# Fireflies-17/Speech-Inpainting

Hardware: AMD Instinct MI355X
Metric: real-time factor (audio-sec/wall-sec) per GPU, 4 s clips @16 kHz, 200 ms mask (higher is better)
Workload: dtype encoder GEMMs and attention products: bf16 MFMA, fp32 accumulate (softmax, LayerNorm, head, arg-max in fp32); vocoder: fp16 MFMA (operands rounded to fp16, saturating), fp32 accumulate, activations stored as fp16; 1 GPU; BASELINE configs[1]: batch=32 x 4 s clips per GPU, 200 ms mask, HuBERT-base + HiFi-GAN V1; step = masked log-mel front-end -> encoder -> arg-max/splice -> vocoder on resident raw clips; global_batch=32, clip_samples=64000, mask_frames=10, parallelism=utterance-sharded x1

## Files before the change

speech_inpainting_amd/csrc/reschain.hip:

```cpp
#include <algorithm>
#include <cstdio>
#include <cstdlib>
#include <type_traits>

#include "common.h"

typedef float f32x4 __attribute__((ext_vector_type(4)));
typedef unsigned int u32x4 __attribute__((ext_vector_type(4)));
typedef unsigned int u32x2 __attribute__((ext_vector_type(2)));
typedef _Float16 f16x8 __attribute__((ext_vector_type(8)));
typedef _Float16 f16x4 __attribute__((ext_vector_type(4)));

#ifdef RPW_TIMELINE
__device__ unsigned long long rc_tl[10];
#define RC_TL_DECL unsigned long long tl_t = wall_clock64(); unsigned long long tl_acc[8] = {0, 0, 0, 0, 0, 0, 0, 0}; unsigned long long tl_tiles = 0; unsigned long long tl_w = 0;
#define RC_TL_W0 tl_w = wall_clock64();
#define RC_TL_W1(ph) tl_acc[ph] += wall_clock64() - tl_w;
#define RC_TL(ph) { const unsigned long long n_ = wall_clock64(); tl_acc[ph] += n_ - tl_t; tl_t = n_; }
#define RC_TL_TILE ++tl_tiles;
#define RC_TL_FLUSH if (threadIdx.x == 0) { for (int q_ = 0; q_ < 8; ++q_) atomicAdd(&rc_tl[q_], tl_acc[q_]); atomicAdd(&rc_tl[8], tl_tiles); atomicAdd(&rc_tl[9], 1ull); }
extern "C" int si_debug_rc_timeline(unsigned long long* out, int reset) {
    if (hipMemcpyFromSymbol(out, HIP_SYMBOL(rc_tl), sizeof(rc_tl)) != hipSuccess) return -1;
    if (reset) { unsigned long long z[10] = {}; if (hipMemcpyToSymbol(HIP_SYMBOL(rc_tl), z, sizeof(z)) != hipSuccess) return -1; }
    return 0;
}
#else
#define RC_TL_DECL
#define RC_TL_W0
#define RC_TL_W1(ph)
#define RC_TL(ph)
#define RC_TL_TILE
#define RC_TL_FLUSH
#endif

namespace {

constexpr int RC_C = 32, RC_ROWB = 64, RC_NW = 8, RC_NT = 64 * RC_NW;
constexpr int RC_RT = 6;
constexpr int RC_R = RC_NW * RC_RT * 16;
constexpr int RC_MARG = 32;
constexpr int RC_KMAX = 11;
constexpr int RC_XBYTES = RC_R * RC_ROWB;
constexpr int RC_ABYTES = (RC_R + 2 * RC_MARG) * RC_ROWB;
constexpr int RC_WBYTES = RC_KMAX * RC_C * RC_ROWB;
constexpr int RC_LDS = RC_XBYTES + RC_ABYTES + 2 * RC_WBYTES + 6 * RC_C * 4;
constexpr int RC_WSLOTS = (RC_WBYTES / 16 + RC_NT - 1) / RC_NT;
constexpr int RC_YSLOTS = RC_R * 4 / RC_NT;
static_assert(RC_R * 4 % RC_NT == 0, "tile staging map");

__device__ __forceinline__ int rc_swz(int row) { return ((row >> 1) & 3) << 4; }

}

template <bool ACC, bool VL>
__global__ __launch_bounds__(RC_NT, 1) void reschain_kernel(const ResChainParams p) {
    extern __shared__ __attribute__((aligned(16))) char smem[];
    char* const Xs = smem;
    char* const As = smem + RC_XBYTES;
    char* const W1s = As + RC_ABYTES;
    char* const W2s = W1s + RC_WBYTES;
    float* const Bs = reinterpret_cast<float*>(W2s + RC_WBYTES);

    __builtin_amdgcn_s_setreg((0 << 11) | (23 << 6) | 1, 1);
    const int tid = threadIdx.x, lane = tid & 63, wave = tid >> 6;
    const int r16 = lane & 15, kg = lane >> 4;
    const int wm0 = wave * (RC_RT * 16);
    const int k = p.k, c = (k - 1) / 2;
    const int H = c * (p.dil[0] + p.dil[1] + p.dil[2] + 3);
    const int Rout = RC_R - 2 * H;
    const int tiles_x = (p.L + Rout - 1) / Rout;
    const int total = VL ? p.total_tiles : tiles_x * p.B;
    auto tile_of = [&](int t, int& tb, int& tm0, int& tL) {
        if constexpr (VL) { const SiVlTile v = si_vl_tile(p.lens, p.B, Rout, t); tb = v.b; tm0 = v.row0; tL = v.L; }
        else { tb = t / tiles_x; tm0 = (t - tb * tiles_x) * Rout; tL = p.L; }
    };
    const int wbytes = k * RC_C * RC_ROWB;

    u32x4 rw[RC_WSLOTS];
    auto issueW = [&](const unsigned short* w) {
        const __amdgpu_buffer_rsrc_t rs = __builtin_amdgcn_make_buffer_rsrc(const_cast<unsigned short*>(w), 0, wbytes, 0x00020000);
// ... 61 lines not shown
            const int lin = lin0 + (tap - c) * dd * RC_ROWB;
            const char* ap = As + (lin ^ ((lin >> 3) & 0x30));
#pragma unroll
            for (int i = 0; i < RC_RT; ++i) y[i] = *reinterpret_cast<const f16x8*>(ap + i * (16 * RC_ROWB));
            const char* wp = Wc + tap * (RC_C * RC_ROWB) + preW;
#pragma unroll
            for (int j = 0; j < 2; ++j) w[j] = *reinterpret_cast<const f16x8*>(wp + j * (16 * RC_ROWB));
        };
        auto mma = [&](const f16x8 (&y)[RC_RT], const f16x8 (&w)[2]) {
#ifdef RC_ABLATE_HALF
            if (wave >= 4) return;
#endif
#ifdef RC_ABLATE_MFMA
#pragma unroll
            for (int i = 0; i < RC_RT; ++i) acc[i][0] += __builtin_bit_cast(f32x4, y[i]);
            acc[0][1] += __builtin_bit_cast(f32x4, w[0]) + __builtin_bit_cast(f32x4, w[1]);
            return;
#endif
#pragma unroll
            for (int i = 0; i < RC_RT; ++i)
#pragma unroll
                for (int j = 0; j < 2; ++j) acc[i][j] = __builtin_amdgcn_mfma_f32_16x16x32_f16(w[j], y[i], acc[i][j], 0, 0, 0);
        };
        f16x8 ya[RC_RT], wa[2], yb[RC_RT], wb[2];
        load(ya, wa, 0);
        for (int tap = 0; tap < k; tap += 2) {
            load(yb, wb, tap + 1 < k ? tap + 1 : k - 1);
            __builtin_amdgcn_sched_barrier(0);
            __builtin_amdgcn_s_setprio(1);
            mma(ya, wa);
            __builtin_amdgcn_s_setprio(0);
            __builtin_amdgcn_sched_barrier(0);
            load(ya, wa, tap + 2 < k ? tap + 2 : k - 1);
            __builtin_amdgcn_sched_barrier(0);
            if (tap + 1 < k) {
                __builtin_amdgcn_s_setprio(1);
                mma(yb, wb);
                __builtin_amdgcn_s_setprio(0);
            }
            __builtin_amdgcn_sched_barrier(0);
        }
    };

    RC_TL_DECL
    for (int tile = blockIdx.x; tile < total; tile += gridDim.x) {
        const int nxt = tile + (int)gridDim.x < total ? tile + (int)gridDim.x : tile;
        int b, tm0, Lb;
        tile_of(tile, b, tm0, Lb);
        const int g0 = tm0 - H;
        const long seg = (long)b * p.L * RC_C;
        const __amdgpu_buffer_rsrc_t orsrc = __builtin_amdgcn_make_buffer_rsrc(p.out16 + seg, 0, Lb * RC_C * 2, 0x00020000);
        const bool edge = g0 < 0 || g0 + RC_R > Lb;

#pragma unroll
        for (int i = 0; i < RC_YSLOTS; ++i) {
            const int q = tid + i * RC_NT;
            const int r = q >> 2, ch = q & 3;
            f16x8 h = __builtin_bit_cast(f16x8, ry[i]);
            *reinterpret_cast<f16x8*>(Xs + r * RC_ROWB + ((ch << 4) ^ rc_swz(r))) = h;
            h = __builtin_elementwise_max(h, h * (_Float16)0.1f);
            const int ra = r + RC_MARG;
            *reinterpret_cast<f16x8*>(As + ra * RC_ROWB + ((ch << 4) ^ rc_swz(ra))) = h;
        }
        __syncthreads();
        RC_TL(0)

        u32x2 prev[ACC ? RC_RT : 1][2];
        auto swap_halves = [&](u32x2& p0, u32x2& p1) {
#pragma unroll
            for (int q = 0; q < 2; ++q) {
                const auto r = __builtin_amdgcn_permlane16_swap(p0[q], p1[q], false, false);
                p0[q] = r[0]; p1[q] = r[1];
            }
        };
        auto chunk_off = [&](int ip, int j, int shift) {
            const int r = wm0 + 16 * (2 * ip + (kg & 1)) + r16 + shift;
            return r * RC_ROWB + ((((2 * j + (kg >> 1)) << 4)) ^ rc_swz(r));
        };
        auto epi1 = [&](auto maskc) {
            constexpr bool MASK = decltype(maskc)::value;
#pragma unroll
            for (int ip = 0; ip < RC_RT / 2; ++ip) {
                float inside[2] = {1.f, 1.f};
                if constexpr (MASK) {
#pragma unroll
                    for (int u = 0; u < 2; ++u) { const int g = g0 + wm0 + 16 * (2 * ip + u) + r16; inside[u] = (g >= 0 && g < Lb) ? 1.f : 0.f; }
                }
#pragma unroll
                for (int j = 0; j < 2; ++j) {
                    u32x2 pk[2];
#pragma unroll
                    for (int u = 0; u < 2; ++u) {
                        f16x4 hv;
#pragma unroll
                        for (int e = 0; e < 4; ++e) {
                            float v = si_lrelu01(acc[2 * ip + u][j][e]);
                            if constexpr (MASK) v *= inside[u];
                            hv[e] = (_Float16)v;
                        }
                        pk[u] = __builtin_bit_cast(u32x2, hv);
                    }
                    swap_halves(pk[0], pk[1]);
                    *reinterpret_cast<u32x4*>(As + chunk_off(ip, j, RC_MARG)) = u32x4{pk[0][0], pk[0][1], pk[1][0], pk[1][1]};
                }
            }
        };
        auto epi2 = [&](auto maskc, auto lastc) {
            constexpr bool MASK = decltype(maskc)::value, LAST = decltype(lastc)::value;
            constexpr int HP = (RC_RT / 2 + 1) / 2;
#pragma unroll
            for (int h = 0; h < 2; ++h) {
                const int ip0 = h * HP, ip1 = h == 0 ? HP : RC_RT / 2;
                f16x4 xr[HP][2][2];
#pragma unroll
                for (int ip = ip0; ip < ip1; ++ip)
#pragma unroll
                    for (int u = 0; u < 2; ++u)
// ... 124 lines not shown
```

speech_inpainting_amd/csrc/respair.hip:

```cpp
#include <algorithm>
#include <cstdio>
#include <cstdlib>
#include <type_traits>

#include "common.h"

typedef float f32x4 __attribute__((ext_vector_type(4)));
typedef unsigned int u32x4 __attribute__((ext_vector_type(4)));
typedef unsigned int u32x2 __attribute__((ext_vector_type(2)));
typedef _Float16 f16x8 __attribute__((ext_vector_type(8)));
typedef _Float16 f16x4 __attribute__((ext_vector_type(4)));

constexpr int RPN_HALO = 50;

template <int ROWB>
__device__ __forceinline__ int rpn_swz(int row) {
    if constexpr (ROWB == 128) return (row & 7) << 4;
    else return ((row >> 1) & 3) << 4;
}

template <int C, int R1, int WARPS_M, int TPS, bool ACC, bool VL>
__global__ __launch_bounds__(64 * WARPS_M, 2) void respair_kernel(const ResPairParams p) {
    static_assert(R1 == WARPS_M * 64 && (C == 32 || C == 64), "64-row wave tiles over all C channels");
    constexpr int NT = 64 * WARPS_M;
    constexpr int ROWB = C * 2;
    constexpr int ROWBO = C * 4;
    constexpr int CPR = C / 8;
    constexpr int KS = C / 32;
    constexpr int TN = C / 16;
    constexpr int YPAD = C == 64 ? 32 : 0;
    constexpr int YS = ROWB + YPAD;
    constexpr int YBYTES = (R1 + RPN_HALO) * YS;
    constexpr int WBYTES = TPS * C * ROWB;
    constexpr int WSLOTS = (WBYTES / 16 + NT - 1) / NT;
    constexpr int YRPP = NT / CPR;
    constexpr int YSLOTS = (R1 + RPN_HALO + YRPP - 1) / YRPP;
    constexpr int OXM = (C / 4 - 1) < 15 ? (C / 4 - 1) : 15;
    static_assert(R1 * ROWBO <= YBYTES + 2 * WBYTES, "the output image reuses the operand region (not the biases behind it)");

    __builtin_amdgcn_s_setreg((0 << 11) | (23 << 6) | 1, 1);
    extern __shared__ __attribute__((aligned(16))) char smem[];
    char* const Ys = smem;
    char* const Ws = smem + YBYTES;
    float* const Bs = reinterpret_cast<float*>(smem + YBYTES + 2 * WBYTES);

    const int tid = threadIdx.x, lane = tid & 63, wave = tid >> 6;
    const int r16 = lane & 15, kg = lane >> 4;
    const int wm0 = wave * 64;
    const int k = p.k, d = p.dil;
    const int p1 = d * (k - 1) / 2, p2 = (k - 1) / 2;
    const int BMo = R1 - (k - 1);
    const int R0 = R1 + (k - 1) * d;
    const int tiles_x = (p.L + BMo - 1) / BMo;
    const int total = VL ? p.total_tiles : tiles_x * p.B;
    auto tile_of = [&](int t, int& tb, int& tm0, int& tL) {
        if constexpr (VL) { const SiVlTile v = si_vl_tile(p.lens, p.B, BMo, t); tb = v.b; tm0 = v.row0; tL = v.L; }
        else { tb = t / tiles_x; tm0 = (t - tb * tiles_x) * BMo; tL = p.L; }
    };
    const __amdgpu_buffer_rsrc_t w1rsrc = __builtin_amdgcn_make_buffer_rsrc(const_cast<unsigned short*>(p.w1), 0, k * C * C * 2, 0x00020000);
    const __amdgpu_buffer_rsrc_t w2rsrc = __builtin_amdgcn_make_buffer_rsrc(const_cast<unsigned short*>(p.w2), 0, k * C * C * 2, 0x00020000);

    const int NS1 = (k + TPS - 1) / TPS, NS = 2 * NS1;
    u32x4 rw[WSLOTS];
    auto issueW = [&](int s) {
        const bool second = s >= NS1;
        const int soff = __builtin_amdgcn_readfirstlane((second ? s - NS1 : s) * WBYTES);
#pragma unroll
        for (int i = 0; i < WSLOTS; ++i)
            rw[i] = __builtin_amdgcn_raw_buffer_load_b128(second ? w2rsrc : w1rsrc, (tid + i * NT) * 16, soff, 0);
    };
    auto storeW = [&](char* dst) {
#pragma unroll
        for (int i = 0; i < WSLOTS; ++i) {
            const int q = tid + i * NT;
            if (WBYTES / 16 % NT == 0 || q < WBYTES / 16) {
                const int r = q / CPR, c = q - r * CPR;
                *reinterpret_cast<u32x4*>(dst + r * ROWB + ((c << 4) ^ rpn_swz<ROWB>(r))) = rw[i];
            }
        }
    };

    const int yc = tid % CPR, yr0 = tid / CPR;
    u32x4 ry[YSLOTS];
    auto issueY = [&](int t) {
        int tb, tm0, tL;
        tile_of(t, tb, tm0, tL);
        const int trow0 = tm0 - p2 - p1;
        const __amdgpu_buffer_rsrc_t rs = __builtin_amdgcn_make_buffer_rsrc(const_cast<unsigned short*>(p.y16 + (long)tb * p.L * C), 0, tL * C * 2, 0x00020000);
#pragma unroll
        for (int i = 0; i < YSLOTS; ++i)
            ry[i] = __builtin_amdgcn_raw_buffer_load_b128(rs, ((trow0 + yr0 + i * YRPP) * C + 8 * yc) * 2, 0, 0);
    };

    issueW(0);
    issueY(blockIdx.x);
    if (tid < C / 2) {
        const int which = tid / (C / 4), c4 = (tid % (C / 4)) * 4;
        *reinterpret_cast<f32x4*>(Bs + which * C + c4) = *reinterpret_cast<const f32x4*>((which ? p.b2 : p.b1) + c4);
    }

  for (int tile = blockIdx.x; tile < total; tile += gridDim.x) {
    const int nxt = tile + (int)gridDim.x < total ? tile + (int)gridDim.x : tile;
    int b, m0, Lb;
    tile_of(tile, b, m0, Lb);
    const int t_row0 = m0 - p2;
    const long seg = (long)b * p.L * C;
    const __amdgpu_buffer_rsrc_t yrsrc = __builtin_amdgcn_make_buffer_rsrc(const_cast<unsigned short*>(p.y16 + seg), 0, Lb * C * 2, 0x00020000);
    const __amdgpu_buffer_rsrc_t orsrc = __builtin_amdgcn_make_buffer_rsrc(p.out16 + seg, 0, Lb * C * 2, 0x00020000);

    storeW(Ws);
    issueW(1);
#pragma unroll
    for (int i = 0; i < YSLOTS; ++i) {
        const int r = yr0 + i * YRPP;
        if ((i + 1) * YRPP <= R1 || r < R0) {
            f16x8 h = __builtin_bit_cast(f16x8, ry[i]);
            h = __builtin_elementwise_max(h, h * (_Float16)0.1f);
            *reinterpret_cast<f16x8*>(Ys + r * YS + (YPAD ? yc << 4 : (yc << 4) ^ rpn_swz<ROWB>(r))) = h;
        }
    }
    __syncthreads();

    f32x4 acc[4][TN];
    auto init_acc = [&](const float* bias) {
#pragma unroll
        for (int j = 0; j < TN; ++j) {
            const f32x4 bv = *reinterpret_cast<const f32x4*>(bias + 16 * j + 4 * kg);
#pragma unroll
            for (int i = 0; i < 4; ++i) acc[i][j] = bv;
        }
    };
    init_acc(Bs);
    const int lin0 = (wm0 + r16) * YS + (kg << 4);
    int preW[KS];
#pragma unroll
    for (int ks = 0; ks < KS; ++ks) preW[ks] = r16 * ROWB + (rpn_swz<ROWB>(r16) ^ (kg << 4) ^ (ks * 64));
    auto compute = [&](int tap0, bool second, int ntap, const char* Wc) {
        const int nsteps = ntap * KS;
        auto load = [&](f16x8 (&y)[4], f16x8 (&w)[TN], int q, const int ks) {
            const int tl = KS == 1 ? q : q >> 1;
            const int soff = (second ? tap0 + tl : (tap0 + tl) * d) * YS + ks * 64;
            const int lin = lin0 + soff;
            const char* yp = Ys + (YPAD ? lin : lin ^ ((lin >> 3) & 0x30));
#pragma unroll
            for (int i = 0; i < 4; ++i) y[i] = *reinterpret_cast<const f16x8*>(yp + i * (16 * YS));
            const char* wp = Wc + tl * (C * ROWB) + preW[ks];
#pragma unroll
            for (int j = 0; j < TN; ++j) w[j] = *reinterpret_cast<const f16x8*>(wp + j * (16 * ROWB));
        };
        auto mma = [&](const f16x8 (&y)[4], const f16x8 (&w)[TN]) {
#pragma unroll
            for (int i = 0; i < 4; ++i)
#pragma unroll
                for (int j = 0; j < TN; ++j) acc[i][j] = __builtin_amdgcn_mfma_f32_16x16x32_f16(w[j], y[i], acc[i][j], 0, 0, 0);
        };
        f16x8 ya[4], wa[TN], yb[4], wb[TN];
        load(ya, wa, 0, 0);
        for (int q = 0; q < nsteps; q += 2) {
            load(yb, wb, q + 1 < nsteps ? q + 1 : nsteps - 1, KS - 1);
            __builtin_amdgcn_sched_barrier(0);
            __builtin_amdgcn_s_setprio(1);
            mma(ya, wa);
            __builtin_amdgcn_s_setprio(0);
            __builtin_amdgcn_sched_barrier(0);
            load(ya, wa, q + 2 < nsteps ? q + 2 : nsteps - KS, 0);
            __builtin_amdgcn_sched_barrier(0);
            if (q + 1 < nsteps) {
                __builtin_amdgcn_s_setprio(1);
                mma(yb, wb);
                __builtin_amdgcn_s_setprio(0);
            }
            __builtin_amdgcn_sched_barrier(0);
        }
    };

    for (int s = 0; s < NS; ++s) {
        const bool second = s >= NS1;
        const int q = second ? s - NS1 : s;
        const int tap0 = q * TPS;
        if (s == NS - 1) {
            issueW(0);
            if constexpr (!ACC) issueY(nxt);
        }
        compute(tap0, second, min(TPS, k - tap0), Ws + (s & 1) * WBYTES);
        if (s == NS1 - 1) {
            __syncthreads();
            auto epi1 = [&](auto edge_tag) {
                constexpr bool EDGE = decltype(edge_tag)::value;
#pragma unroll
            for (int ip = 0; ip < 2; ++ip) {
                float inside[2];
#pragma unroll
                for (int u = 0; u < 2; ++u) {
                    const int grow = t_row0 + wm0 + 16 * (2 * ip + u) + r16;
                    inside[u] = (!EDGE || (grow >= 0 && grow < Lb)) ? 1.f : 0.f;
                }
                const int ms = wm0 + 16 * (2 * ip + (kg & 1)) + r16;
#pragma unroll
                for (int j = 0; j < TN; ++j) {
                    u32x2 pk[2];
#pragma unroll
                    for (int u = 0; u < 2; ++u) {
                        f16x4 hv;
#pragma unroll
                        for (int e = 0; e < 4; ++e) hv[e] = (_Float16)(EDGE ? si_lrelu01(acc[2 * ip + u][j][e]) * inside[u] : si_lrelu01(acc[2 * ip + u][j][e]));
                        pk[u] = __builtin_bit_cast(u32x2, hv);
                    }
#pragma unroll
                    for (int q = 0; q < 2; ++q) {
                        const auto r = __builtin_amdgcn_permlane16_swap(pk[0][q], pk[1][q], false, false);
                        pk[0][q] = r[0]; pk[1][q] = r[1];
                    }
                    const int ch = 2 * j + (kg >> 1);
                    *reinterpret_cast<u32x4*>(Ys + ms * YS + (YPAD ? ch << 4 : (ch << 4) ^ rpn_swz<ROWB>(ms))) = u32x4{pk[0][0], pk[0][1], pk[1][0], pk[1][1]};
                }
            }
            };
            if (t_row0 >= 0 && t_row0 + R1 <= Lb) epi1(std::false_type{});
            else epi1(std::true_type{});
            init_acc(Bs + C);
        }
        if (s + 1 < NS) {
            storeW(Ws + ((s + 1) & 1) * WBYTES);
            if (s + 2 < NS) issueW(s + 2);
        }
        __syncthreads();
    }

    constexpr int ORPP = NT / CPR;
    constexpr int OPASS = R1 / ORPP;
    const int c8 = tid % CPR, or0 = tid / CPR;
    u32x4 res[OPASS], prev[ACC ? OPASS : 1];
    int goff[OPASS];
#pragma unroll
    for (int it = 0; it < OPASS; ++it) {
        const int o = or0 + it * ORPP;
        const int grow = m0 + o;
        goff[it] = (o < BMo && grow < Lb) ? (grow * C + 8 * c8) * 2 : (int)0x80000000;
        res[it] = __builtin_amdgcn_raw_buffer_load_b128(yrsrc, goff[it], 0, 0);
        if constexpr (ACC) prev[it] = __builtin_amdgcn_raw_buffer_load_b128(orsrc, goff[it], 0, 0);
    }
#pragma unroll
    for (int i = 0; i < 4; ++i) {
        const int m = wm0 + 16 * i + r16;
#pragma unroll
        for (int j = 0; j < TN; ++j) {
            const int co = 4 * j + kg;
            *reinterpret_cast<f32x4*>(smem + m * ROWBO + ((co ^ (m & OXM)) << 4)) = acc[i][j];
        }
    }
    __syncthreads();
    {
#pragma unroll
        for (int it = 0; it < OPASS; ++it) {
            const int o = or0 + it * ORPP;
            const f32x4 a0 = *reinterpret_cast<const f32x4*>(smem + o * ROWBO + (((2 * c8) ^ (o & OXM)) << 4));
            const f32x4 a1 = *reinterpret_cast<const f32x4*>(smem + o * ROWBO + (((2 * c8 + 1) ^ (o & OXM)) << 4));
            const f16x8 rh = __builtin_bit_cast(f16x8, res[it]);
            f16x8 ph = {};
            if constexpr (ACC) ph = __builtin_bit_cast(f16x8, prev[it]);
            f16x8 out;
#pragma unroll
            for (int e = 0; e < 8; ++e) {
                const float a = e < 4 ? a0[e] : a1[e - 4];
                float v = (a + (float)rh[e]) * p.alpha;
                if constexpr (ACC) v += (float)ph[e];
                out[e] = (_Float16)v;
            }
            __builtin_amdgcn_raw_buffer_store_b128(__builtin_bit_cast(u32x4, out), orsrc, goff[it], 0, 0);
        }
    }
    if constexpr (ACC) issueY(nxt);
    __syncthreads();
  }
}

template <int C, int R1, int WARPS_M, int TPS>
static int respair_launch(si_ctx* ctx, const ResPairParams& p, hipStream_t st) {
    const int BMo = R1 - (p.k - 1);
    const size_t lds = (size_t)(R1 + RPN_HALO) * (C * 2 + (C == 64 ? 32 : 0)) + 2 * (size_t)TPS * C * C * 2 + 2 * (size_t)C * 4;
    const bool vl = p.lens != nullptr;
    auto kern = vl ? (p.accumulate ? respair_kernel<C, R1, WARPS_M, TPS, true, true> : respair_kernel<C, R1, WARPS_M, TPS, false, true>)
                   : (p.accumulate ? respair_kernel<C, R1, WARPS_M, TPS, true, false> : respair_kernel<C, R1, WARPS_M, TPS, false, false>);
    if (int rc = si_ensure_dyn_lds(ctx, reinterpret_cast<const void*>(kern), lds)) return rc;
    const int total = vl ? (int)si_vl_tiles(p.lens_host, p.B, BMo) : ((p.L + BMo - 1) / BMo) * p.B;
    if (total <= 0) return SI_OK;
    ResPairParams pk = p;
    pk.total_tiles = total;
    const int grid = std::min(total, si_num_cus(ctx) * (WARPS_M == 4 ? 2 : 1));
    char name[48];
    snprintf(name, sizeof(name), p.accumulate ? "respair_f16_c%d_acc" : "respair_f16_c%d", C);
    double rows = (double)p.B * p.L;
    if (vl) { rows = 0; for (int b = 0; b < p.B; ++b) rows += p.lens_host[b]; }
    const double elems = rows * C;
    si_prof_begin(ctx, name, 2.0 * 2.0 * elems * C * p.k, elems * (2.0 + 2.0 + (p.accumulate ? 2.0 : 0.0)) + 2.0 * 2.0 * p.k * C * C, st);
    hipLaunchKernelGGL(kern, dim3(grid), dim3(64 * WARPS_M), lds, st, pk);
    si_prof_end(ctx, st);
    SI_HIP_CHECK(hipGetLastError());
    return SI_OK;
}

int si_launch_respair(si_ctx* ctx, int C, const unsigned short* y16, unsigned short* out16, const void* w1, const void* w2,
                      const float* b1, const float* b2, int B, int L, int k, int dil, float alpha, int accumulate, hipStream_t st,
                      const int32_t* lens, const int32_t* lens_host, float out_slope) {
    if ((C != 32 && C != 64 && C != 128 && C != 256) || k < 3 || k > 11 || (k & 1) == 0 || (k - 1) * dil > 50 ||
        ((long)L + 1024) * C * 2 >= (1L << 31)) return 1;
    if (!b1 || !b2) return 1;
    if ((lens == nullptr) != (lens_host == nullptr)) return si_fail(ctx, SI_EINVAL, "respair: ragged batches need the lengths on the device and on the host");
    ResPairParams p{y16, out16, static_cast<const unsigned short*>(w1), static_cast<const unsigned short*>(w2), b1, b2, B, L, k, dil, alpha, accumulate, lens, lens_host, 0, out_slope};
    if (out_slope != 1.f && C < 128) return 1;
    if (C >= 128) return si_launch_respair_wide(ctx, C, p, st);
    return C == 32 ? respair_launch<32, 256, 4, 11>(ctx, p, st) : respair_launch<64, 512, 8, 4>(ctx, p, st);
}
```

speech_inpainting_amd/csrc/respair_wide.hip:

```cpp
#include <algorithm>
#include <cstdio>
#include <cstdlib>

#include "common.h"

typedef float f32x4 __attribute__((ext_vector_type(4)));
typedef unsigned int u32x4 __attribute__((ext_vector_type(4)));
typedef unsigned int u32x2 __attribute__((ext_vector_type(2)));
typedef _Float16 f16x8 __attribute__((ext_vector_type(8)));
typedef _Float16 f16x4 __attribute__((ext_vector_type(4)));

template <int ROWB>
__device__ __forceinline__ int swz16(int row) {
    if constexpr (ROWB >= 256) return (row & 7) << 5;
    else return ((row >> 1) & 3) << 5;
}

#ifdef RPW_TIMELINE
__device__ unsigned long long rpw_tl[2][10];
#define RPW_TL_DECL unsigned long long tl_t = wall_clock64(); unsigned long long tl_acc[6] = {0, 0, 0, 0, 0, 0}; unsigned long long tl_tiles = 0; unsigned long long tl_w = 0, tl_sub[2] = {0, 0};
#define RPW_TL_W0 tl_w = wall_clock64();
#define RPW_TL_W1(q) tl_sub[q] += wall_clock64() - tl_w;
#define RPW_TL(ph) { const unsigned long long n_ = wall_clock64(); tl_acc[ph] += n_ - tl_t; tl_t = n_; }
#define RPW_TL_TILE ++tl_tiles;
#define RPW_TL_FLUSH if (threadIdx.x == 0) { for (int q_ = 0; q_ < 6; ++q_) atomicAdd(&rpw_tl[C == 256][q_], tl_acc[q_]); atomicAdd(&rpw_tl[C == 256][6], tl_tiles); atomicAdd(&rpw_tl[C == 256][7], 1ull); atomicAdd(&rpw_tl[C == 256][8], tl_sub[0]); atomicAdd(&rpw_tl[C == 256][9], tl_sub[1]); }
extern "C" int si_debug_rpw_timeline(unsigned long long* out, int reset) {
    if (hipMemcpyFromSymbol(out, HIP_SYMBOL(rpw_tl), sizeof(rpw_tl)) != hipSuccess) return -1;
    if (reset) { unsigned long long z[2][10] = {}; if (hipMemcpyToSymbol(HIP_SYMBOL(rpw_tl), z, sizeof(z)) != hipSuccess) return -1; }
    return 0;
}
#else
#define RPW_TL_DECL
#define RPW_TL_W0
#define RPW_TL_W1(q)
#define RPW_TL(ph)
#define RPW_TL_TILE
#define RPW_TL_FLUSH
#endif

constexpr int RPW_HALO = 50;

template <int C, int R1, int WARPS_M, int WARPS_N, int BKW, bool ACC, bool VL>
__global__ __launch_bounds__(64 * WARPS_M * WARPS_N, 2) void respair_wide_kernel(const ResPairParams p) {
    static_assert((WARPS_M * WARPS_N == 8 || WARPS_M * WARPS_N == 4) && R1 == WARPS_M * 64 && C == WARPS_N * 64, "64 x 64 wave tiles");
    static_assert(BKW == 128 || BKW == 64, "weight-slab depth");
    constexpr int NT = 64 * WARPS_M * WARPS_N;
    constexpr int ROWBY = C * 2;
    constexpr int ROWBW = BKW * 2;
    constexpr int ROWBO = C * 4;
    constexpr int CPRY = C / 8, CPRW = BKW / 8;
    constexpr int NCH = C / BKW;
    constexpr int KS = BKW / 32;
    constexpr int YBYTES = (R1 + RPW_HALO) * ROWBY;
    constexpr int WBYTES = C * ROWBW;
    constexpr int WSLOTS = C * CPRW / NT;
    constexpr int YSLOTS = ((R1 + RPW_HALO) * CPRY + NT - 1) / NT;
    constexpr int YRPP = NT / CPRY, WRPP = NT / CPRW;
    static_assert(C * CPRW % NT == 0 && NT % CPRY == 0 && NT % CPRW == 0, "staging maps");
    static_assert(R1 * ROWBO <= YBYTES + 2 * WBYTES, "the output image reuses the operand region (not the biases behind it)");

    __builtin_amdgcn_s_setreg((0 << 11) | (23 << 6) | 1, 1);
    extern __shared__ __attribute__((aligned(16))) char smem[];
    char* const Ys = smem;
    char* const Ws = smem + YBYTES;
    float* const Bs = reinterpret_cast<float*>(smem + YBYTES + 2 * WBYTES);

    const int tid = threadIdx.x, lane = tid & 63, wave = tid >> 6;
    const int r16 = lane & 15, kg = lane >> 4;
    const int wm0 = (wave / WARPS_N) * 64, wn0 = (wave % WARPS_N) * 64;
    const int k = p.k, d = p.dil;
    const int p1 = d * (k - 1) / 2, p2 = (k - 1) / 2;
    const int BMo = R1 - (k - 1);
    const int R0 = R1 + (k - 1) * d;
    const int tiles_x = (p.L + BMo - 1) / BMo;
    const int total = VL ? p.total_tiles : tiles_x * p.B;
    auto tile_of = [&](int t, int& tb, int& tm0, int& tL) {
        if constexpr (VL) { const SiVlTile v = si_vl_tile(p.lens, p.B, BMo, t); tb = v.b; tm0 = v.row0; tL = v.L; }
        else { tb = t / tiles_x; tm0 = (t - tb * tiles_x) * BMo; tL = p.L; }
    };
    const __amdgpu_buffer_rsrc_t w1rsrc = __builtin_amdgcn_make_buffer_rsrc(const_cast<unsigned short*>(p.w1), 0, k * C * C * 2, 0x00020000);
    const __amdgpu_buffer_rsrc_t w2rsrc = __builtin_amdgcn_make_buffer_rsrc(const_cast<unsigned short*>(p.w2), 0, k * C * C * 2, 0x00020000);

    const int NS1 = k * NCH, NS = 2 * NS1;
    const int wc = tid % CPRW, wr0 = tid / CPRW;
    u32x4 rw[WSLOTS];
    auto issueW1 = [&](int s, int i) {
        const bool second = s >= NS1;
        const int q = second ? s - NS1 : s;
        const int tap = q / NCH, ch = q - tap * NCH;
        const int soff = __builtin_amdgcn_readfirstlane((tap * C * C + ch * BKW) * 2);
        const int n = wr0 + i * WRPP;
        rw[i] = __builtin_amdgcn_raw_buffer_load_b128(second ? w2rsrc : w1rsrc, (n * C + 8 * wc) * 2, soff, 0);
    };
    auto issueW = [&](int s) {
#pragma unroll
        for (int i = 0; i < WSLOTS; ++i) issueW1(s, i);
    };
    auto storeW1 = [&](char* dst, int i) {
        const int n = wr0 + i * WRPP;
        *reinterpret_cast<u32x4*>(dst + n * ROWBW + ((wc << 4) ^ swz16<ROWBW>(n))) = rw[i];
    };
    auto storeW = [&](char* dst) {
#pragma unroll
        for (int i = 0; i < WSLOTS; ++i) storeW1(dst, i);
    };
    const int yc = tid % CPRY, yr0 = tid / CPRY;
    u32x4 ry[YSLOTS];
    auto issueY = [&](int t) {
        int tb, tm0, tL;
        tile_of(t, tb, tm0, tL);
        const int trow0 = tm0 - p2 - p1;
        const __amdgpu_buffer_rsrc_t rs = __builtin_amdgcn_make_buffer_rsrc(const_cast<unsigned short*>(p.y16 + (long)tb * p.L * C), 0, tL * C * 2, 0x00020000);
#pragma unroll
        for (int i = 0; i < YSLOTS; ++i)
            ry[i] = __builtin_amdgcn_raw_buffer_load_b128(rs, ((trow0 + yr0 + i * YRPP) * C + 8 * yc) * 2, 0, 0);
    };

    if (tid < C / 2) {
        const int which = tid / (C / 4), c4 = (tid % (C / 4)) * 4;
        *reinterpret_cast<f32x4*>(Bs + which * C + c4) = *reinterpret_cast<const f32x4*>((which ? p.b2 : p.b1) + c4);
    }
    const int preW = (wn0 + r16) * ROWBW + (swz16<ROWBW>(wn0 + r16) ^ (kg << 4));
    issueW(0);
    issueY(blockIdx.x);
    RPW_TL_DECL

  for (int tile = blockIdx.x; tile < total; tile += gridDim.x) {
    const int nxt = tile + (int)gridDim.x < total ? tile + (int)gridDim.x : tile;
    int b, m0, Lb;
    tile_of(tile, b, m0, Lb);
    const int t_row0 = m0 - p2;
    const long seg = (long)b * p.L * C;
    const __amdgpu_buffer_rsrc_t yrsrc = __builtin_amdgcn_make_buffer_rsrc(const_cast<unsigned short*>(p.y16 + seg), 0, Lb * C * 2, 0x00020000);
    const __amdgpu_buffer_rsrc_t orsrc = __builtin_amdgcn_make_buffer_rsrc(p.out16 + seg, 0, Lb * C * 2, 0x00020000);

    storeW(Ws);
    issueW(1);
#pragma unroll
    for (int i = 0; i < YSLOTS; ++i) {
        const int r = yr0 + i * YRPP;
        if ((i + 1) * YRPP <= R1 || r < R0) {
            f16x8 h = __builtin_bit_cast(f16x8, ry[i]);
            h = __builtin_elementwise_max(h, h * (_Float16)0.1f);
            *reinterpret_cast<f16x8*>(Ys + r * ROWBY + ((yc << 4) ^ swz16<ROWBY>(r))) = h;
        }
    }
    __syncthreads();
    RPW_TL(0)

    f32x4 acc[4][4];
    auto init_acc = [&](const float* bias) {
#pragma unroll
        for (int j = 0; j < 4; ++j) {
            const f32x4 bv = *reinterpret_cast<const f32x4*>(bias + wn0 + 16 * j + 4 * kg);
#pragma unroll
            for (int i = 0; i < 4; ++i) acc[i][j] = bv;
        }
    };
    init_acc(Bs);
    auto compute = [&](int roff, int cb16, const char* Wc, auto&& hook) {
        const int r0 = wm0 + r16 + roff;
        const int preY = r0 * ROWBY + (swz16<ROWBY>(r0) ^ (kg << 4));
        auto load = [&](f16x8 (&y)[4], f16x8 (&w)[4], int ks) {
            const char* yp = Ys + (preY ^ (cb16 + ks * 64));
            const char* wp = Wc + (preW ^ (ks * 64));
#pragma unroll
            for (int i = 0; i < 4; ++i) y[i] = *reinterpret_cast<const f16x8*>(yp + i * (16 * ROWBY));
#pragma unroll
            for (int j = 0; j < 4; ++j) w[j] = *reinterpret_cast<const f16x8*>(wp + j * (16 * ROWBW));
        };
        auto mma = [&](const f16x8 (&y)[4], const f16x8 (&w)[4]) {
#pragma unroll
            for (int i = 0; i < 4; ++i)
#pragma unroll
                for (int j = 0; j < 4; ++j) acc[i][j] = __builtin_amdgcn_mfma_f32_16x16x32_f16(w[j], y[i], acc[i][j], 0, 0, 0);
        };
        f16x8 ya[4], wa[4], yb[4], wb[4];
        load(ya, wa, 0);
#pragma unroll
        for (int ks = 0; ks < KS; ks += 2) {
            load(yb, wb, ks + 1);
            __builtin_amdgcn_sched_barrier(0);
            __builtin_amdgcn_s_setprio(1);
            mma(ya, wa);
            __builtin_amdgcn_s_setprio(0);
            __builtin_amdgcn_sched_barrier(0);
            hook(ks);
            if (ks + 2 < KS) load(ya, wa, ks + 2);
            __builtin_amdgcn_sched_barrier(0);
            __builtin_amdgcn_s_setprio(1);
            mma(yb, wb);
            __builtin_amdgcn_s_setprio(0);
            __builtin_amdgcn_sched_barrier(0);
            hook(ks + 1);
        }
    };

    int tap = 0, ch = 0;
    for (int s = 0; s < NS - 1; ++s) {
        const bool second = s >= NS1;
        char* const Wn = Ws + ((s + 1) & 1) * WBYTES;
        static_assert(WSLOTS % KS == 0, "the slab's stores are spread evenly over its k-steps");
        compute(second ? tap : tap * d, ch * (BKW * 2), Ws + (s & 1) * WBYTES, [&](int ks) {
            const int s2 = s + 2 < NS ? s + 2 : NS - 1;
#pragma unroll
            for (int i = 0; i < WSLOTS / KS; ++i) {
                storeW1(Wn, ks * (WSLOTS / KS) + i);
                issueW1(s2, ks * (WSLOTS / KS) + i);
            }
        });
        if (s == NS1 - 1) {
            __syncthreads();
            RPW_TL(1)
#pragma unroll
            for (int ip = 0; ip < 2; ++ip) {
                float inside[2];
#pragma unroll
                for (int u = 0; u < 2; ++u) {
                    const int grow = t_row0 + wm0 + 16 * (2 * ip + u) + r16;
                    inside[u] = (grow >= 0 && grow < Lb) ? 1.f : 0.f;
                }
                const int ms = wm0 + 16 * (2 * ip + (kg & 1)) + r16;
#pragma unroll
                for (int j = 0; j < 4; ++j) {
                    u32x2 pk[2];
#pragma unroll
                    for (int u = 0; u < 2; ++u) {
                        f16x4 hv;
#pragma unroll
                        for (int e = 0; e < 4; ++e) hv[e] = (_Float16)(si_lrelu01(acc[2 * ip + u][j][e]) * inside[u]);
                        pk[u] = __builtin_bit_cast(u32x2, hv);
                    }
#pragma unroll
                    for (int q = 0; q < 2; ++q) {
                        const auto r = __builtin_amdgcn_permlane16_swap(pk[0][q], pk[1][q], false, false);
                        pk[0][q] = r[0]; pk[1][q] = r[1];
                    }
                    const int ch = ((wn0 + 16 * j) >> 3) + (kg >> 1);
                    *reinterpret_cast<u32x4*>(Ys + ms * ROWBY + ((ch << 4) ^ swz16<ROWBY>(ms))) = u32x4{pk[0][0], pk[0][1], pk[1][0], pk[1][1]};
                }
            }
            init_acc(Bs + C);
            RPW_TL(2)
        }
        if (++ch == NCH) { ch = 0; if (++tap == k) tap = 0; }
        __syncthreads();
    }
    if constexpr (!ACC) issueY(nxt);
    __builtin_amdgcn_sched_barrier(0);
    compute(tap, ch * (BKW * 2), Ws + ((NS - 1) & 1) * WBYTES, [](int) {});
    RPW_TL(3)
    constexpr int ORPP = NT / CPRY;
    constexpr int OPASS = R1 / ORPP;
    const int c8 = tid % CPRY, or0 = tid / CPRY;
    u32x4 res[OPASS], prev[ACC ? OPASS : 1];
    int goff[OPASS];
#pragma unroll
    for (int it = 0; it < OPASS; ++it) {
        const int o = or0 + it * ORPP;
        const int grow = m0 + o;
        goff[it] = (o < BMo && grow < Lb) ? (grow * C + 8 * c8) * 2 : (int)0x80000000;
        res[it] = __builtin_amdgcn_raw_buffer_load_b128(yrsrc, goff[it], 0, 0);
        if constexpr (ACC) prev[it] = __builtin_amdgcn_raw_buffer_load_b128(orsrc, goff[it], 0, 0);
    }
    RPW_TL_W0
    __syncthreads();
    RPW_TL_W1(0)
    RPW_TL_W0

#pragma unroll
    for (int i = 0; i < 4; ++i) {
        const int m = wm0 + 16 * i + r16;
#pragma unroll
        for (int j = 0; j < 4; ++j) {
            const int co = ((wn0 + 16 * j) >> 2) + kg;
            *reinterpret_cast<f32x4*>(smem + m * ROWBO + ((co ^ (m & 15)) << 4)) = acc[i][j];
        }
    }
    RPW_TL_W1(1)
    __syncthreads();
    RPW_TL(4)
    issueW(0);
    {
        const bool oact = p.out_slope != 0.f && p.out_slope != 1.f;
#pragma unroll
        for (int it = 0; it < OPASS; ++it) {
            const int o = or0 + it * ORPP;
            const f32x4 a0 = *reinterpret_cast<const f32x4*>(smem + o * ROWBO + (((2 * c8) ^ (o & 15)) << 4));
            const f32x4 a1 = *reinterpret_cast<const f32x4*>(smem + o * ROWBO + (((2 * c8 + 1) ^ (o & 15)) << 4));
            const f16x8 rh = __builtin_bit_cast(f16x8, res[it]);
            f16x8 ph = {};
            if constexpr (ACC) ph = __builtin_bit_cast(f16x8, prev[it]);
            f16x8 out;
#pragma unroll
            for (int e = 0; e < 8; ++e) {
                const float a = e < 4 ? a0[e] : a1[e - 4];
                float v = (a + (float)rh[e]) * p.alpha;
                if constexpr (ACC) v += (float)ph[e];
                if (oact) v = v > 0.f ? v : v * p.out_slope;
                out[e] = (_Float16)v;
            }
            __builtin_amdgcn_raw_buffer_store_b128(__builtin_bit_cast(u32x4, out), orsrc, goff[it], 0, 0);
        }
    }
    if constexpr (ACC) issueY(nxt);
    __syncthreads();
    RPW_TL(5)
    RPW_TL_TILE
  }
  RPW_TL_FLUSH
}

template <int C, int R1, int WARPS_M, int WARPS_N, int BKW>
static int respair_wide_launch(si_ctx* ctx, const ResPairParams& p0, hipStream_t st) {
    const ResPairParams& p = p0;
    const int BMo = R1 - (p.k - 1);
    const size_t lds = (size_t)(R1 + RPW_HALO) * C * 2 + 2 * (size_t)C * BKW * 2 + 2 * (size_t)C * 4;
    const bool vl = p0.lens != nullptr;
    auto kern = vl ? (p.accumulate ? respair_wide_kernel<C, R1, WARPS_M, WARPS_N, BKW, true, true> : respair_wide_kernel<C, R1, WARPS_M, WARPS_N, BKW, false, true>)
                   : (p.accumulate ? respair_wide_kernel<C, R1, WARPS_M, WARPS_N, BKW, true, false> : respair_wide_kernel<C, R1, WARPS_M, WARPS_N, BKW, false, false>);
    if (int rc = si_ensure_dyn_lds(ctx, reinterpret_cast<const void*>(kern), lds)) return rc;
    const int total = vl ? (int)si_vl_tiles(p.lens_host, p.B, BMo) : ((p.L + BMo - 1) / BMo) * p.B;
    if (total <= 0) return SI_OK;
    ResPairParams pk = p0;
    pk.total_tiles = total;
    const int grid = std::min(total, si_num_cus(ctx) * (WARPS_M * WARPS_N == 4 ? 2 : 1));
    char name[48];
    snprintf(name, sizeof(name), p.accumulate ? "respair_f16_c%d_acc" : "respair_f16_c%d", C);
    double rows = (double)p.B * p.L;
    if (vl) { rows = 0; for (int b = 0; b < p.B; ++b) rows += p.lens_host[b]; }
    const double elems = rows * C;
    si_prof_begin(ctx, name, 2.0 * 2.0 * elems * C * p.k, elems * (2.0 + 2.0 + (p.accumulate ? 2.0 : 0.0)) + 2.0 * 2.0 * p.k * C * C, st);
    hipLaunchKernelGGL(kern, dim3(grid), dim3(64 * WARPS_M * WARPS_N), lds, st, pk);
    si_prof_end(ctx, st);
    SI_HIP_CHECK(hipGetLastError());
    return SI_OK;
}

int si_launch_respair_wide(si_ctx* ctx, int C, const ResPairParams& p, hipStream_t st) {
    if (C == 128) return respair_wide_launch<128, 256, 4, 2, 128>(ctx, p, st);
    if (C == 256) return respair_wide_launch<256, 128, 2, 4, 64>(ctx, p, st);
    return 1;
}
```

Baseline: 10790 x real-time (audio-sec/wall-sec); `value` = whole-job aggregate over n_gpus, `value_per_gpu` = the per-GPU figure the metric names.

## Prefetch next tile earlier in residual-pair kernels and split accumulate epilogue loads

In respair, the next tile's activation prefetch (issueY) now always starts before the last weight slab, not after the epilogue for the accumulate variant. The accumulate epilogue now loads residual and previous-output rows in two halves, so fewer registers are live while the early prefetch is in flight. respair_wide does the same for the non-accumulate and C==128 accumulate paths. Tile coordinates are made wave-uniform with readfirstlane, and timeline-only stage counters are added under a debug macro. The risk is higher register pressure or extra exposed epilogue latency from the split loads.

New measurement: 10850 x real-time (audio-sec/wall-sec); `value` = whole-job aggregate over n_gpus, `value_per_gpu` = the per-GPU figure the metric names, median of 6. No clear change (+0.6%).

```diff
diff --git a/speech_inpainting_amd/csrc/reschain.hip b/speech_inpainting_amd/csrc/reschain.hip
--- a/speech_inpainting_amd/csrc/reschain.hip
+++ b/speech_inpainting_amd/csrc/reschain.hip
@@ -13,19 +13,31 @@
 
 #ifdef RPW_TIMELINE
 __device__ unsigned long long rc_tl[10];
-#define RC_TL_DECL unsigned long long tl_t = wall_clock64(); unsigned long long tl_acc[8] = {0, 0, 0, 0, 0, 0, 0, 0}; unsigned long long tl_tiles = 0; unsigned long long tl_w = 0;
+__device__ unsigned long long rc_stage[2][3][5];
+#define RC_TL_DECL unsigned long long tl_t = wall_clock64(); unsigned long long tl_acc[8] = {0, 0, 0, 0, 0, 0, 0, 0}; unsigned long long tl_tiles = 0; unsigned long long tl_w = 0; unsigned long long st_acc[4] = {0, 0, 0, 0}, st_t0 = 0;
+#define RC_TL_YWAIT(reg) { const unsigned w_ = __builtin_amdgcn_readfirstlane((reg)[0]); asm volatile("" :: "s"(w_)); st_t0 = tl_t; if (tile != (int)blockIdx.x) st_acc[0] += wall_clock64() - tl_t; }
+#define RC_TL_STAGED if (tile != (int)blockIdx.x) { st_acc[1] += wall_clock64() - tl_t; ++st_acc[2]; }
 #define RC_TL_W0 tl_w = wall_clock64();
 #define RC_TL_W1(ph) tl_acc[ph] += wall_clock64() - tl_w;
 #define RC_TL(ph) { const unsigned long long n_ = wall_clock64(); tl_acc[ph] += n_ - tl_t; tl_t = n_; }
-#define RC_TL_TILE ++tl_tiles;
-#define RC_TL_FLUSH if (threadIdx.x == 0) { for (int q_ = 0; q_ < 8; ++q_) atomicAdd(&rc_tl[q_], tl_acc[q_]); atomicAdd(&rc_tl[8], tl_tiles); atomicAdd(&rc_tl[9], 1ull); }
+#define RC_TL_TILE ++tl_tiles; if (tile != (int)blockIdx.x) st_acc[3] += tl_t - st_t0;
+#define RC_TL_FLUSH if (threadIdx.x == 0) { for (int q_ = 0; q_ < 8; ++q_) atomicAdd(&rc_tl[q_], tl_acc[q_]); atomicAdd(&rc_tl[8], tl_tiles); atomicAdd(&rc_tl[9], 1ull); \
+    for (int q_ = 0; q_ < 4; ++q_) atomicAdd(&rc_stage[ACC][(p.k - 3) >> 2][q_], st_acc[q_]); } \
+    if ((threadIdx.x & 63) == 0) atomicAdd(&rc_stage[ACC][(p.k - 3) >> 2][4], st_acc[0]);
 extern "C" int si_debug_rc_timeline(unsigned long long* out, int reset) {
     if (hipMemcpyFromSymbol(out, HIP_SYMBOL(rc_tl), sizeof(rc_tl)) != hipSuccess) return -1;
     if (reset) { unsigned long long z[10] = {}; if (hipMemcpyToSymbol(HIP_SYMBOL(rc_tl), z, sizeof(z)) != hipSuccess) return -1; }
     return 0;
 }
+extern "C" int si_debug_rc_stage(unsigned long long* out, int reset) {
+    if (hipMemcpyFromSymbol(out, HIP_SYMBOL(rc_stage), sizeof(rc_stage)) != hipSuccess) return -1;
+    if (reset) { unsigned long long z[2][3][5] = {}; if (hipMemcpyToSymbol(HIP_SYMBOL(rc_stage), z, sizeof(z)) != hipSuccess) return -1; }
+    return 0;
+}
 #else
 #define RC_TL_DECL
+#define RC_TL_YWAIT(reg)
+#define RC_TL_STAGED
 #define RC_TL_W0
 #define RC_TL_W1(ph)
 #define RC_TL(ph)
@@ -193,6 +205,7 @@
         const __amdgpu_buffer_rsrc_t orsrc = __builtin_amdgcn_make_buffer_rsrc(p.out16 + seg, 0, Lb * RC_C * 2, 0x00020000);
         const bool edge = g0 < 0 || g0 + RC_R > Lb;
 
+        RC_TL_YWAIT(ry[RC_YSLOTS - 1])
 #pragma unroll
         for (int i = 0; i < RC_YSLOTS; ++i) {
             const int q = tid + i * RC_NT;
@@ -204,6 +217,7 @@
             *reinterpret_cast<f16x8*>(As + ra * RC_ROWB + ((ch << 4) ^ rc_swz(ra))) = h;
         }
         __syncthreads();
+        RC_TL_STAGED
         RC_TL(0)
 
         u32x2 prev[ACC ? RC_RT : 1][2];
diff --git a/speech_inpainting_amd/csrc/respair.hip b/speech_inpainting_amd/csrc/respair.hip
--- a/speech_inpainting_amd/csrc/respair.hip
+++ b/speech_inpainting_amd/csrc/respair.hip
@@ -18,6 +18,27 @@
     if constexpr (ROWB == 128) return (row & 7) << 4;
     else return ((row >> 1) & 3) << 4;
 }
+
+#ifdef RPW_TIMELINE
+__device__ unsigned long long rpn_stage[2][2][3][5];
+#define RPN_TL_DECL unsigned long long tl_t = wall_clock64(), st_acc[4] = {0, 0, 0, 0};
+#define RPN_TL_YWAIT(reg) { const unsigned w_ = __builtin_amdgcn_readfirstlane((reg)[0]); asm volatile("" :: "s"(w_)); if (tile != (int)blockIdx.x) st_acc[0] += wall_clock64() - tl_t; }
+#define RPN_TL_STAGED if (tile != (int)blockIdx.x) { st_acc[1] += wall_clock64() - tl_t; ++st_acc[2]; }
+#define RPN_TL_TILE { const unsigned long long n_ = wall_clock64(); if (tile != (int)blockIdx.x) st_acc[3] += n_ - tl_t; tl_t = n_; }
+#define RPN_TL_FLUSH if (threadIdx.x == 0) { for (int q_ = 0; q_ < 4; ++q_) atomicAdd(&rpn_stage[C == 64][ACC][(p.k - 3) >> 2][q_], st_acc[q_]); } \
+    if ((threadIdx.x & 63) == 0) atomicAdd(&rpn_stage[C == 64][ACC][(p.k - 3) >> 2][4], st_acc[0]);
+extern "C" int si_debug_rpn_stage(unsigned long long* out, int reset) {
+    if (hipMemcpyFromSymbol(out, HIP_SYMBOL(rpn_stage), sizeof(rpn_stage)) != hipSuccess) return -1;
+    if (reset) { unsigned long long z[2][2][3][5] = {}; if (hipMemcpyToSymbol(HIP_SYMBOL(rpn_stage), z, sizeof(z)) != hipSuccess) return -1; }
+    return 0;
+}
+#else
+#define RPN_TL_DECL
+#define RPN_TL_YWAIT(reg)
+#define RPN_TL_STAGED
+#define RPN_TL_TILE
+#define RPN_TL_FLUSH
+#endif
 
 template <int C, int R1, int WARPS_M, int TPS, bool ACC, bool VL>
 __global__ __launch_bounds__(64 * WARPS_M, 2) void respair_kernel(const ResPairParams p) {
@@ -54,7 +75,10 @@
     const int tiles_x = (p.L + BMo - 1) / BMo;
     const int total = VL ? p.total_tiles : tiles_x * p.B;
     auto tile_of = [&](int t, int& tb, int& tm0, int& tL) {
-        if constexpr (VL) { const SiVlTile v = si_vl_tile(p.lens, p.B, BMo, t); tb = v.b; tm0 = v.row0; tL = v.L; }
+        if constexpr (VL) {
+            const SiVlTile v = si_vl_tile(p.lens, p.B, BMo, t);
+            tb = __builtin_amdgcn_readfirstlane(v.b); tm0 = __builtin_amdgcn_readfirstlane(v.row0); tL = __builtin_amdgcn_readfirstlane(v.L);
+        }
         else { tb = t / tiles_x; tm0 = (t - tb * tiles_x) * BMo; tL = p.L; }
     };
     const __amdgpu_buffer_rsrc_t w1rsrc = __builtin_amdgcn_make_buffer_rsrc(const_cast<unsigned short*>(p.w1), 0, k * C * C * 2, 0x00020000);
@@ -98,6 +122,7 @@
         const int which = tid / (C / 4), c4 = (tid % (C / 4)) * 4;
         *reinterpret_cast<f32x4*>(Bs + which * C + c4) = *reinterpret_cast<const f32x4*>((which ? p.b2 : p.b1) + c4);
     }
+    RPN_TL_DECL
 
   for (int tile = blockIdx.x; tile < total; tile += gridDim.x) {
     const int nxt = tile + (int)gridDim.x < total ? tile + (int)gridDim.x : tile;
@@ -108,6 +133,7 @@
     const __amdgpu_buffer_rsrc_t yrsrc = __builtin_amdgcn_make_buffer_rsrc(const_cast<unsigned short*>(p.y16 + seg), 0, Lb * C * 2, 0x00020000);
     const __amdgpu_buffer_rsrc_t orsrc = __builtin_amdgcn_make_buffer_rsrc(p.out16 + seg, 0, Lb * C * 2, 0x00020000);
 
+    RPN_TL_YWAIT(ry[YSLOTS - 1])
     storeW(Ws);
     issueW(1);
 #pragma unroll
@@ -120,6 +146,7 @@
         }
     }
     __syncthreads();
+    RPN_TL_STAGED
 
     f32x4 acc[4][TN];
     auto init_acc = [&](const float* bias) {
@@ -174,16 +201,15 @@
         }
     };
 
-    for (int s = 0; s < NS; ++s) {
+    auto slab = [&](int s, auto pos) {
+        constexpr int POS = decltype(pos)::value;
         const bool second = s >= NS1;
         const int q = second ? s - NS1 : s;
         const int tap0 = q * TPS;
-        if (s == NS - 1) {
-            issueW(0);
-            if constexpr (!ACC) issueY(nxt);
-        }
+        if constexpr (POS == 1) issueY(nxt);
+        if constexpr (POS == 2) issueW(0);
         compute(tap0, second, min(TPS, k - tap0), Ws + (s & 1) * WBYTES);
-        if (s == NS1 - 1) {
+        if (POS != 2 && s == NS1 - 1) {
             __syncthreads();
             auto epi1 = [&](auto edge_tag) {
                 constexpr bool EDGE = decltype(edge_tag)::value;
@@ -220,25 +246,32 @@
             else epi1(std::true_type{});
             init_acc(Bs + C);
         }
-        if (s + 1 < NS) {
+        if constexpr (POS != 2) {
             storeW(Ws + ((s + 1) & 1) * WBYTES);
-            if (s + 2 < NS) issueW(s + 2);
+            if constexpr (POS == 0) issueW(s + 2);
         }
         __syncthreads();
-    }
+    };
+    for (int s = 0; s < NS - 2; ++s) slab(s, std::integral_constant<int, 0>{});
+    slab(NS - 2, std::integral_constant<int, 1>{});
+    slab(NS - 1, std::integral_constant<int, 2>{});
 
     constexpr int ORPP = NT / CPR;
     constexpr int OPASS = R1 / ORPP;
+    constexpr int OHALF = ACC ? OPASS / 2 : OPASS;
+    static_assert(OPASS % 2 == 0, "the accumulate variant's two halves");
     const int c8 = tid % CPR, or0 = tid / CPR;
-    u32x4 res[OPASS], prev[ACC ? OPASS : 1];
+    u32x4 res[OHALF], prev[ACC ? OHALF : 1];
     int goff[OPASS];
 #pragma unroll
     for (int it = 0; it < OPASS; ++it) {
         const int o = or0 + it * ORPP;
         const int grow = m0 + o;
         goff[it] = (o < BMo && grow < Lb) ? (grow * C + 8 * c8) * 2 : (int)0x80000000;
-        res[it] = __builtin_amdgcn_raw_buffer_load_b128(yrsrc, goff[it], 0, 0);
-        if constexpr (ACC) prev[it] = __builtin_amdgcn_raw_buffer_load_b128(orsrc, goff[it], 0, 0);
+        if (it < OHALF) {
+            res[it] = __builtin_amdgcn_raw_buffer_load_b128(yrsrc, goff[it], 0, 0);
+            if constexpr (ACC) prev[it] = __builtin_amdgcn_raw_buffer_load_b128(orsrc, goff[it], 0, 0);
+        }
     }
 #pragma unroll
     for (int i = 0; i < 4; ++i) {
@@ -256,9 +289,15 @@
             const int o = or0 + it * ORPP;
             const f32x4 a0 = *reinterpret_cast<const f32x4*>(smem + o * ROWBO + (((2 * c8) ^ (o & OXM)) << 4));
             const f32x4 a1 = *reinterpret_cast<const f32x4*>(smem + o * ROWBO + (((2 * c8 + 1) ^ (o & OXM)) << 4));
-            const f16x8 rh = __builtin_bit_cast(f16x8, res[it]);
+            const f16x8 rh = __builtin_bit_cast(f16x8, res[it % OHALF]);
             f16x8 ph = {};
-            if constexpr (ACC) ph = __builtin_bit_cast(f16x8, prev[it]);
+            if constexpr (ACC) {
+                ph = __builtin_bit_cast(f16x8, prev[it % OHALF]);
+                if (it + OHALF < OPASS) {
+                    res[it % OHALF] = __builtin_amdgcn_raw_buffer_load_b128(yrsrc, goff[it + OHALF], 0, 0);
+                    prev[it % OHALF] = __builtin_amdgcn_raw_buffer_load_b128(orsrc, goff[it + OHALF], 0, 0);
+                }
+            }
             f16x8 out;
 #pragma unroll
             for (int e = 0; e < 8; ++e) {
@@ -270,9 +309,10 @@
             __builtin_amdgcn_raw_buffer_store_b128(__builtin_bit_cast(u32x4, out), orsrc, goff[it], 0, 0);
         }
     }
-    if constexpr (ACC) issueY(nxt);
     __syncthreads();
+    RPN_TL_TILE
   }
+  RPN_TL_FLUSH
 }
 
 template <int C, int R1, int WARPS_M, int TPS>
diff --git a/speech_inpainting_amd/csrc/respair_wide.hip b/speech_inpainting_amd/csrc/respair_wide.hip
--- a/speech_inpainting_amd/csrc/respair_wide.hip
+++ b/speech_inpainting_amd/csrc/respair_wide.hip
@@ -18,19 +18,31 @@
 
 #ifdef RPW_TIMELINE
 __device__ unsigned long long rpw_tl[2][10];
-#define RPW_TL_DECL unsigned long long tl_t = wall_clock64(); unsigned long long tl_acc[6] = {0, 0, 0, 0, 0, 0}; unsigned long long tl_tiles = 0; unsigned long long tl_w = 0, tl_sub[2] = {0, 0};
+__device__ unsigned long long rpw_stage[2][2][3][5];
+#define RPW_TL_DECL unsigned long long tl_t = wall_clock64(); unsigned long long tl_acc[6] = {0, 0, 0, 0, 0, 0}; unsigned long long tl_tiles = 0; unsigned long long tl_w = 0, tl_sub[2] = {0, 0}; unsigned long long st_acc[4] = {0, 0, 0, 0}, st_t0 = 0;
+#define RPW_TL_YWAIT(reg) { const unsigned w_ = __builtin_amdgcn_readfirstlane((reg)[0]); asm volatile("" :: "s"(w_)); st_t0 = tl_t; if (tile != (int)blockIdx.x) st_acc[0] += wall_clock64() - tl_t; }
+#define RPW_TL_STAGED if (tile != (int)blockIdx.x) { st_acc[1] += wall_clock64() - tl_t; ++st_acc[2]; }
 #define RPW_TL_W0 tl_w = wall_clock64();
 #define RPW_TL_W1(q) tl_sub[q] += wall_clock64() - tl_w;
 #define RPW_TL(ph) { const unsigned long long n_ = wall_clock64(); tl_acc[ph] += n_ - tl_t; tl_t = n_; }
-#define RPW_TL_TILE ++tl_tiles;
-#define RPW_TL_FLUSH if (threadIdx.x == 0) { for (int q_ = 0; q_ < 6; ++q_) atomicAdd(&rpw_tl[C == 256][q_], tl_acc[q_]); atomicAdd(&rpw_tl[C == 256][6], tl_tiles); atomicAdd(&rpw_tl[C == 256][7], 1ull); atomicAdd(&rpw_tl[C == 256][8], tl_sub[0]); atomicAdd(&rpw_tl[C == 256][9], tl_sub[1]); }
+#define RPW_TL_TILE ++tl_tiles; if (tile != (int)blockIdx.x) st_acc[3] += tl_t - st_t0;
+#define RPW_TL_FLUSH if (threadIdx.x == 0) { for (int q_ = 0; q_ < 6; ++q_) atomicAdd(&rpw_tl[C == 256][q_], tl_acc[q_]); atomicAdd(&rpw_tl[C == 256][6], tl_tiles); atomicAdd(&rpw_tl[C == 256][7], 1ull); atomicAdd(&rpw_tl[C == 256][8], tl_sub[0]); atomicAdd(&rpw_tl[C == 256][9], tl_sub[1]); \
+    for (int q_ = 0; q_ < 4; ++q_) atomicAdd(&rpw_stage[C == 256][ACC][(p.k - 3) >> 2][q_], st_acc[q_]); } \
+    if ((threadIdx.x & 63) == 0) atomicAdd(&rpw_stage[C == 256][ACC][(p.k - 3) >> 2][4], st_acc[0]);
 extern "C" int si_debug_rpw_timeline(unsigned long long* out, int reset) {
     if (hipMemcpyFromSymbol(out, HIP_SYMBOL(rpw_tl), sizeof(rpw_tl)) != hipSuccess) return -1;
     if (reset) { unsigned long long z[2][10] = {}; if (hipMemcpyToSymbol(HIP_SYMBOL(rpw_tl), z, sizeof(z)) != hipSuccess) return -1; }
     return 0;
 }
+extern "C" int si_debug_rpw_stage(unsigned long long* out, int reset) {
+    if (hipMemcpyFromSymbol(out, HIP_SYMBOL(rpw_stage), sizeof(rpw_stage)) != hipSuccess) return -1;
+    if (reset) { unsigned long long z[2][2][3][5] = {}; if (hipMemcpyToSymbol(HIP_SYMBOL(rpw_stage), z, sizeof(z)) != hipSuccess) return -1; }
+    return 0;
+}
 #else
 #define RPW_TL_DECL
+#define RPW_TL_YWAIT(reg)
+#define RPW_TL_STAGED
 #define RPW_TL_W0
 #define RPW_TL_W1(q)
 #define RPW_TL(ph)
@@ -58,6 +70,7 @@
     constexpr int YRPP = NT / CPRY, WRPP = NT / CPRW;
     static_assert(C * CPRW % NT == 0 && NT % CPRY == 0 && NT % CPRW == 0, "staging maps");
     static_assert(R1 * ROWBO <= YBYTES + 2 * WBYTES, "the output image reuses the operand region (not the biases behind it)");
+    constexpr bool YEARLY = !ACC || C == 128;
 
     __builtin_amdgcn_s_setreg((0 << 11) | (23 << 6) | 1, 1);
     extern __shared__ __attribute__((aligned(16))) char smem[];
@@ -75,7 +88,10 @@
     const int tiles_x = (p.L + BMo - 1) / BMo;
     const int total = VL ? p.total_tiles : tiles_x * p.B;
     auto tile_of = [&](int t, int& tb, int& tm0, int& tL) {
-        if constexpr (VL) { const SiVlTile v = si_vl_tile(p.lens, p.B, BMo, t); tb = v.b; tm0 = v.row0; tL = v.L; }
+        if constexpr (VL) {
+            const SiVlTile v = si_vl_tile(p.lens, p.B, BMo, t);
+            tb = __builtin_amdgcn_readfirstlane(v.b); tm0 = __builtin_amdgcn_readfirstlane(v.row0); tL = __builtin_amdgcn_readfirstlane(v.L);
+        }
         else { tb = t / tiles_x; tm0 = (t - tb * tiles_x) * BMo; tL = p.L; }
     };
     const __amdgpu_buffer_rsrc_t w1rsrc = __builtin_amdgcn_make_buffer_rsrc(const_cast<unsigned short*>(p.w1), 0, k * C * C * 2, 0x00020000);
@@ -134,6 +150,7 @@
     const __amdgpu_buffer_rsrc_t yrsrc = __builtin_amdgcn_make_buffer_rsrc(const_cast<unsigned short*>(p.y16 + seg), 0, Lb * C * 2, 0x00020000);
     const __amdgpu_buffer_rsrc_t orsrc = __builtin_amdgcn_make_buffer_rsrc(p.out16 + seg, 0, Lb * C * 2, 0x00020000);
 
+    RPW_TL_YWAIT(ry[YSLOTS - 1])
     storeW(Ws);
     issueW(1);
 #pragma unroll
@@ -146,6 +163,7 @@
         }
     }
     __syncthreads();
+    RPW_TL_STAGED
     RPW_TL(0)
 
     f32x4 acc[4][4];
@@ -246,22 +264,26 @@
         if (++ch == NCH) { ch = 0; if (++tap == k) tap = 0; }
         __syncthreads();
     }
-    if constexpr (!ACC) issueY(nxt);
+    if constexpr (YEARLY) issueY(nxt);
     __builtin_amdgcn_sched_barrier(0);
     compute(tap, ch * (BKW * 2), Ws + ((NS - 1) & 1) * WBYTES, [](int) {});
     RPW_TL(3)
     constexpr int ORPP = NT / CPRY;
     constexpr int OPASS = R1 / ORPP;
+    constexpr int OHALF = ACC && YEARLY ? OPASS / 2 : OPASS;
+    static_assert(OPASS % 2 == 0, "the accumulate variant's two halves");
     const int c8 = tid % CPRY, or0 = tid / CPRY;
-    u32x4 res[OPASS], prev[ACC ? OPASS : 1];
+    u32x4 res[OHALF], prev[ACC ? OHALF : 1];
     int goff[OPASS];
 #pragma unroll
     for (int it = 0; it < OPASS; ++it) {
         const int o = or0 + it * ORPP;
         const int grow = m0 + o;
         goff[it] = (o < BMo && grow < Lb) ? (grow * C + 8 * c8) * 2 : (int)0x80000000;
-        res[it] = __builtin_amdgcn_raw_buffer_load_b128(yrsrc, goff[it], 0, 0);
-        if constexpr (ACC) prev[it] = __builtin_amdgcn_raw_buffer_load_b128(orsrc, goff[it], 0, 0);
+        if (it < OHALF) {
+            res[it] = __builtin_amdgcn_raw_buffer_load_b128(yrsrc, goff[it], 0, 0);
+            if constexpr (ACC) prev[it] = __builtin_amdgcn_raw_buffer_load_b128(orsrc, goff[it], 0, 0);
+        }
     }
     RPW_TL_W0
     __syncthreads();
@@ -288,9 +310,15 @@
             const int o = or0 + it * ORPP;
             const f32x4 a0 = *reinterpret_cast<const f32x4*>(smem + o * ROWBO + (((2 * c8) ^ (o & 15)) << 4));
             const f32x4 a1 = *reinterpret_cast<const f32x4*>(smem + o * ROWBO + (((2 * c8 + 1) ^ (o & 15)) << 4));
-            const f16x8 rh = __builtin_bit_cast(f16x8, res[it]);
+            const f16x8 rh = __builtin_bit_cast(f16x8, res[it % OHALF]);
             f16x8 ph = {};
-            if constexpr (ACC) ph = __builtin_bit_cast(f16x8, prev[it]);
+            if constexpr (ACC) {
+                ph = __builtin_bit_cast(f16x8, prev[it % OHALF]);
+                if (it + OHALF < OPASS) {
+                    res[it % OHALF] = __builtin_amdgcn_raw_buffer_load_b128(yrsrc, goff[it + OHALF], 0, 0);
+                    prev[it % OHALF] = __builtin_amdgcn_raw_buffer_load_b128(orsrc, goff[it + OHALF], 0, 0);
+                }
+            }
             f16x8 out;
 #pragma unroll
             for (int e = 0; e < 8; ++e) {
@@ -303,7 +331,7 @@
             __builtin_amdgcn_raw_buffer_store_b128(__builtin_bit_cast(u32x4, out), orsrc, goff[it], 0, 0);
         }
     }
-    if constexpr (ACC) issueY(nxt);
+    if constexpr (!YEARLY) issueY(nxt);
     __syncthreads();
     RPW_TL(5)
     RPW_TL_TILE
```
